# talmolab/sleap

Hardware: NVIDIA H100
Metric: frames/sec (1024x1024 bottom-up UNet+PAF) (higher is better)
Workload: dtype f16

## Files before the change

sleap_b200/csrc/sb_conv_tc.cu:

```cuda
#include <cuda.h>

#include <algorithm>

#include "sb_model.h"

namespace {

constexpr int TW = 16, TH = 8;
constexpr int MAX_GROUPS = 7, MAX_TAPS = 7;
constexpr size_t kMaxDynSmem = 225 * 1024;

struct TcTap { int row_off, w_tap; };
struct TcGroup { int dx, n_taps; TcTap taps[MAX_TAPS]; };

struct TcParams {
  int H, W;
  int tiles_x;
  int n_chunks, KC;
  int n_groups;
  TcGroup groups[MAX_GROUPS];
  int dy0, box_rows;
  int N, Cout;
  void* out;
  int out_f32, out_H, out_W, out_Ctot, out_coff;
// ... 466 lines not shown

  const int wg = warp >> 2;
  float acc[N / 2];
  const uint64_t desc_hi = make_desc(0, P.row_bytes, P.layout_type);
  const uint32_t a_row0 = (uint32_t)(wg * 64 * P.row_bytes);
  const uint32_t b_base = smem_u32(bank);
  mbar_wait(smem_u32(fullB), 0);
  int sa = 0;
  uint32_t pha = 0;
  for (int w = blockIdx.x; w < n_work; w += gridDim.x) {
    const int tile = w % P.n_tiles, b = w / P.n_tiles;
    const int x0 = (tile % P.tiles_x) * TW, y0 = (tile / P.tiles_x) * TH;
#pragma unroll
    for (int i = 0; i < N / 2; ++i) acc[i] = 0.f;
    int rel_a = -1, s = 0;
    uint32_t scale_d = 0;
    for (int ch = 0; ch < P.n_chunks; ++ch) {
      for (int g = 0; g < P.n_groups; ++g) {
        mbar_wait(smem_u32(fullA + sa), pha);
        const uint32_t a_base = smem_u32(a_ring + (size_t)sa * P.a_slot_bytes) + a_row0;
        const int n_taps = P.groups[g].n_taps;
        for (int t = 0; t < n_taps; ++t, ++s) {
          const uint64_t da = desc_hi + (uint64_t)((a_base + (uint32_t)(P.groups[g].taps[t].row_off * TW * P.row_bytes)) >> 4);
          const uint64_t db = desc_hi + (uint64_t)((b_base + (uint32_t)(s * P.b_slot_bytes)) >> 4);
          wgmma_fence();
          wgmma_reg_fence(acc);
#pragma unroll
          for (int k = 0; k < KSTEPS; ++k) {
            wgmma_f16<N>(acc, da + 2 * k, db + 2 * k, scale_d);
            scale_d = 1;
          }
          wgmma_commit();
          wgmma_reg_fence(acc);
          wgmma_wait<1>();
          __syncwarp();
          if (lane == 0 && rel_a >= 0) mbar_arrive(smem_u32(emptyA + rel_a));
          rel_a = t == n_taps - 1 ? sa : -1;
        }
        if (++sa == P.n_a_slots) { sa = 0; pha ^= 1; }
      }
    }
    wgmma_wait<0>();
    wgmma_reg_fence(acc);
    __syncwarp();
    if (lane == 0) mbar_arrive(smem_u32(emptyA + rel_a));
    if (w != (int)blockIdx.x) consumer_sync();
    conv_epilogue<N>(P, s_par, s_stage, acc, x0, y0, 0, b, warp, lane);
  }
}

constexpr int kHaloCols = 18;
constexpr int halo_by(int n, int kc) { return n <= 32 && n * kc <= 1024 ? 2 : 1; }
constexpr int halo_plane(int n, int kc) { return (8 * halo_by(n, kc) + 2) * kHaloCols * 16; }
constexpr int kHaloThreads = 384;

template <int NP>
__device__ __forceinline__ void stage_halo_patch(const TcParams& P, uint32_t dst, int plane, int rows, int c0, int b, int ys, int xs,
                                                 int lid, int n_loaders) {
  const __half* in = reinterpret_cast<const __half*>(P.in);
  const int pl = lid % NP, c = c0 + pl * 8;
  const bool c_ok = c < P.in_C;
  const __half* in_c = in + (size_t)b * P.H * P.W * P.in_Ctot + c;
  const uint32_t d = dst + (uint32_t)(pl * plane);
  for (int p = lid / NP; p < rows * kHaloCols; p += n_loaders / NP) {
    const int y = ys + p / kHaloCols, x = xs + p % kHaloCols;
    const bool ok = c_ok && y >= 0 && y < P.H && x >= 0 && x < P.W;
    const __half* src = ok ? in_c + ((size_t)y * P.W + x) * P.in_Ctot : in;
    asm volatile("cp.async.cg.shared.global [%0], [%1], 16, %2;" ::"r"(d + (uint32_t)(p * 16)), "l"(src), "r"(ok ? 16 : 0) : "memory");
  }
}

__device__ __forceinline__ void quad_transpose(uint32_t& v0, uint32_t& v1, uint32_t& v2, uint32_t& v3, int t) {
  const bool o1 = t & 1, o2 = t & 2;
  uint32_t r = __shfl_xor_sync(0xffffffffu, o1 ? v0 : v1, 1);
  if (o1) v0 = r; else v1 = r;
  r = __shfl_xor_sync(0xffffffffu, o1 ? v2 : v3, 1);
  if (o1) v2 = r; else v3 = r;
  r = __shfl_xor_sync(0xffffffffu, o2 ? v0 : v2, 2);
  if (o2) v0 = r; else v2 = r;
  r = __shfl_xor_sync(0xffffffffu, o2 ? v1 : v3, 2);
  if (o2) v1 = r; else v3 = r;
}

__device__ __forceinline__ uint32_t hmax2_u32(uint32_t a, uint32_t b) {
  const __half2 m = __hmax2(*reinterpret_cast<const __half2*>(&a), *reinterpret_cast<const __half2*>(&b));
  return *reinterpret_cast<const uint32_t*>(&m);
}

__device__ __forceinline__ float2 lds_f2(uint32_t saddr) {
  float2 v;
  asm("ld.shared.v2.f32 {%0, %1}, [%2];" : "=f"(v.x), "=f"(v.y) : "r"(saddr));
  return v;
}

template <int N>
__device__ __forceinline__ void frag_rows_f16(const float (&acc)[N / 2], uint32_t s_bias, int t, float lo, uint32_t (&hv)[N / 4]) {
  constexpr int NJ = N / 8;
#pragma unroll
  for (int j = 0; j < NJ; ++j) {
    const float2 bb = lds_f2(s_bias + 4u * (8 * j + 2 * t));
#pragma unroll
    for (int r = 0; r < 2; ++r) {
      const __half2 h2 = __floats2half2_rn(fmaxf(acc[4 * j + 2 * r] + bb.x, lo), fmaxf(acc[4 * j + 2 * r + 1] + bb.y, lo));
      hv[r * NJ + j] = *reinterpret_cast<const uint32_t*>(&h2);
    }
  }
}

template <int N>
__device__ __forceinline__ void frag_rows_store(uint32_t (&hv)[N / 4], __half* po, size_t row_step, bool ok0, bool ok1, int t) {
  constexpr int NJ = N / 8;
#pragma unroll
  for (int c0 = 0; c0 < 2 * NJ; c0 += 4) {
    quad_transpose(hv[c0], hv[c0 + 1], hv[c0 + 2], hv[c0 + 3], t);
    const int c = c0 + t, r = c / NJ, j = c % NJ;
    if (r ? ok1 : ok0) *reinterpret_cast<uint4*>(po + r * row_step + 8 * j) = make_uint4(hv[c0], hv[c0 + 1], hv[c0 + 2], hv[c0 + 3]);
  }
}

template <int N>
__device__ __forceinline__ void halo_block_epilogue(const TcParams& P, const float (&acc)[N / 2], uint32_t s_bias, int n0, int b,
                                                    int y, int x, int g, int t, float lo) {
  constexpr int NJ = N / 8;
  uint32_t hv[2 * NJ];
  frag_rows_f16<N>(acc, s_bias, t, lo, hv);
  if (P.pool_out != nullptr) {
    constexpr int NJ4 = (NJ + 3) / 4 * 4;
    uint32_t pv[NJ4];
#pragma unroll
    for (int j = 0; j < NJ4; ++j) {
      if (j < NJ) {
        const uint32_t m0 = hmax2_u32(hv[j], __shfl_xor_sync(0xffffffffu, hv[j], 4));
        const uint32_t m1 = hmax2_u32(hv[NJ + j], __shfl_xor_sync(0xffffffffu, hv[NJ + j], 4));
        pv[j] = hmax2_u32(m0, m1);
      } else {
        pv[j] = 0u;
      }
    }
    __half* pp = reinterpret_cast<__half*>(P.pool_out) + (((size_t)b * P.pool_H + (y >> 1)) * P.pool_W + (x >> 1)) * P.pool_Ctot +
                 P.pool_coff + n0;
    const bool st = (g & 1) == 0 && y < P.H && x < P.W;
#pragma unroll
    for (int c0 = 0; c0 < NJ4; c0 += 4) {
      quad_transpose(pv[c0], pv[c0 + 1], pv[c0 + 2], pv[c0 + 3], t);
      if (st && c0 + t < NJ) *reinterpret_cast<uint4*>(pp + 8 * (c0 + t)) = make_uint4(pv[c0], pv[c0 + 1], pv[c0 + 2], pv[c0 + 3]);
    }
  }
  if (!P.skip_out) {
    __half* po = reinterpret_cast<__half*>(P.out) + (((size_t)b * P.out_H + y) * P.out_W + x) * P.out_Ctot + P.out_coff + n0;
    frag_rows_store<N>(hv, po, (size_t)P.out_W * P.out_Ctot, y < P.H && x < P.W, y + 1 < P.H && x < P.W, t);
  }
}

template <int KSTEPS, int N>
__global__ void __launch_bounds__(kHaloThreads, 1) k_conv_wg_h(const __grid_constant__ CUtensorMap mapA,
                                                               const __grid_constant__ CUtensorMap mapB,
                                                               const __grid_constant__ TcParams P) {
  constexpr int BY = halo_by(N, 16 * KSTEPS), NB = 2 * BY;
  constexpr int NP = 2 * KSTEPS;
  constexpr int PH = 8 * BY + 2, PW = kHaloCols, PLANE = halo_plane(N, 16 * KSTEPS), SLOT = NP * PLANE;
  constexpr int kLoaders = kHaloThreads - kConsumerThreads;
  extern __shared__ __align__(1024) uint8_t smem_raw[];
  uint8_t* base = reinterpret_cast<uint8_t*>((reinterpret_cast<uintptr_t>(smem_raw) + 1023) & ~(uintptr_t)1023);
  uint8_t* bank = base;
  uint8_t* ring = bank + 9 * (size_t)P.b_slot_bytes;
  uint64_t* full = reinterpret_cast<uint64_t*>(ring + (size_t)P.n_a_slots * SLOT);
  uint64_t* empty = full + P.n_a_slots;
  uint64_t* fullB = empty + P.n_a_slots;
  float* s_bias = reinterpret_cast<float*>(fullB + 1);

  const int warp = threadIdx.x >> 5, lane = threadIdx.x & 31;
  const int tiles_x = (P.W + 15) / 16, n_tiles = tiles_x * ((P.H + 8 * BY - 1) / (8 * BY));
  const int n_work = n_tiles * P.batch;
  for (int i = threadIdx.x; i < N; i += blockDim.x) s_bias[i] = (P.bias && i < P.Cout) ? P.bias[i] : 0.f;
  if (threadIdx.x == 0) {
    for (int i = 0; i < P.n_a_slots; ++i) { mbar_init(smem_u32(full + i), kLoaders); mbar_init(smem_u32(empty + i), 4); }
    mbar_init(smem_u32(fullB), 1);
    asm volatile("fence.mbarrier_init.release.cluster;" ::: "memory");
    asm volatile("prefetch.tensormap [%0];" ::"l"(&mapB) : "memory");
  }
  __syncthreads();

  if (warp < kLoaders / 32) {
    if (threadIdx.x == 0) {
      mbar_expect_tx(smem_u32(fullB), (uint32_t)(9 * P.b_tx_bytes));
      for (int kx = 0; kx < 3; ++kx)
        for (int ky = 0; ky < 3; ++ky)
          tma_load_3d(smem_u32(bank + (size_t)(kx * 3 + ky) * P.b_slot_bytes), &mapB, smem_u32(fullB), 0, 0, ky * 3 + kx);
    }
    griddep_wait();
    for (int i = 0, w = blockIdx.x; w < n_work; ++i, w += gridDim.x) {
      if (w + (int)gridDim.x >= n_work) griddep_launch();
      const int s = i % P.n_a_slots;
      mbar_wait(smem_u32(empty + s), ((i / P.n_a_slots) & 1) ^ 1);
      const int tile = w % n_tiles, b = w / n_tiles;
      stage_halo_patch<NP>(P, smem_u32(ring + (size_t)s * SLOT), PLANE, PH, 0, b, (tile / tiles_x) * (8 * BY) - 1,
                           (tile % tiles_x) * 16 - 1, threadIdx.x, kLoaders);
      asm volatile("cp.async.mbarrier.arrive.noinc.shared::cta.b64 [%0];" ::"r"(smem_u32(full + s)) : "memory");
    }
    asm volatile("cp.async.wait_all;" ::: "memory");
    return;
  }

  const int wg = (warp >> 2) - 1, q = warp & 3, g = lane >> 2, t = lane & 3;
  const float lo = P.relu ? 0.f : -INFINITY;
  const uint64_t desc_a = make_desc_interleave(0, PLANE, PW * 16);
  const uint64_t desc_b = make_desc(0, P.row_bytes, P.layout_type);
  const uint32_t b_base = smem_u32(bank);
  mbar_wait(smem_u32(fullB), 0);
  float acc[NB][N / 2];
  for (int i = wg, w = blockIdx.x + wg * (int)gridDim.x; w < n_work; i += 2, w += 2 * (int)gridDim.x) {
    const int s = i % P.n_a_slots;
    mbar_wait(smem_u32(full + s), (i / P.n_a_slots) & 1);
    asm volatile("fence.proxy.async.shared::cta;" ::: "memory");
    const uint32_t a_base = smem_u32(ring + (size_t)s * SLOT);
    wgmma_fence();
#pragma unroll
    for (int bk = 0; bk < NB; ++bk) wgmma_reg_fence(acc[bk]);
#pragma unroll
    for (int kx = 0; kx < 3; ++kx)
#pragma unroll
      for (int ky = 0; ky < 3; ++ky)
#pragma unroll
        for (int k = 0; k < KSTEPS; ++k) {
          const uint64_t db = desc_b + (uint64_t)((b_base + (uint32_t)((kx * 3 + ky) * P.b_slot_bytes)) >> 4) + 2 * k;
#pragma unroll
          for (int bk = 0; bk < NB; ++bk) {
            const uint32_t a = a_base + (uint32_t)(((8 * (bk >> 1) + ky) * PW + 8 * (bk & 1) + kx) * 16 + 2 * k * PLANE);
            wgmma_f16<N>(acc[bk], desc_a + (uint64_t)(a >> 4), db, (kx | ky | k) ? 1u : 0u);
          }
        }
    wgmma_commit();
#pragma unroll
    for (int bk = 0; bk < NB; ++bk) wgmma_reg_fence(acc[bk]);
    wgmma_wait<0>();
#pragma unroll
    for (int bk = 0; bk < NB; ++bk) wgmma_reg_fence(acc[bk]);
    __syncwarp();
    if (lane == 0) mbar_arrive(smem_u32(empty + s));

    const int tile = w % n_tiles, b = w / n_tiles;
    const int x0 = (tile % tiles_x) * 16, y0 = (tile / tiles_x) * (8 * BY);
#pragma unroll
    for (int bk = 0; bk < NB; ++bk)
      halo_block_epilogue<N>(P, acc[bk], smem_u32(s_bias), 0, b, y0 + 8 * (bk >> 1) + 2 * q, x0 + 8 * (bk & 1) + g, g, t, lo);
  }
}

constexpr int kWideThreads = 384;
constexpr int kWidePatchLoaders = 96;
constexpr int wide_by(int n) { return n <= 64 ? 4 : 2; }
constexpr int wide_plane(int n) { return (8 * wide_by(n) + 2) * kHaloCols * 16; }

template <int N>
__global__ void __launch_bounds__(kWideThreads, 1) k_conv_wg_hw(const __grid_constant__ CUtensorMap mapA,
                                                                const __grid_constant__ CUtensorMap mapB,
                                                                const __grid_constant__ TcParams P) {
  constexpr int BY = wide_by(N), NP = 8, PH = 8 * BY + 2, PW = kHaloCols, PLANE = wide_plane(N), SLOT = NP * PLANE;
  constexpr int WSLOT = N * 128;
  extern __shared__ __align__(1024) uint8_t smem_raw[];
  uint8_t* base = reinterpret_cast<uint8_t*>((reinterpret_cast<uintptr_t>(smem_raw) + 1023) & ~(uintptr_t)1023);
  uint8_t* wring = base;
  uint8_t* pring = wring + (size_t)P.n_b_slots * WSLOT;
  uint64_t* pfull = reinterpret_cast<uint64_t*>(pring + (size_t)P.n_a_slots * SLOT);
  uint64_t* pempty = pfull + P.n_a_slots;
  uint64_t* wfull = pempty + P.n_a_slots;
  uint64_t* wempty = wfull + P.n_b_slots;
  float* s_bias = reinterpret_cast<float*>(wempty + P.n_b_slots);

  const int warp = threadIdx.x >> 5, lane = threadIdx.x & 31;
  const int tiles_x = (P.W + 15) / 16, n_pt = tiles_x * ((P.H + 8 * BY - 1) / (8 * BY));
  const int n_nt = P.Cout / N, n_work = n_nt * n_pt * P.batch;
  for (int i = threadIdx.x; i < P.Cout; i += blockDim.x) s_bias[i] = P.bias ? P.bias[i] : 0.f;
  if (threadIdx.x == 0) {
    for (int i = 0; i < P.n_a_slots; ++i) { mbar_init(smem_u32(pfull + i), kWidePatchLoaders); mbar_init(smem_u32(pempty + i), 8); }
    for (int i = 0; i < P.n_b_slots; ++i) { mbar_init(smem_u32(wfull + i), 1); mbar_init(smem_u32(wempty + i), 8); }
    asm volatile("fence.mbarrier_init.release.cluster;" ::: "memory");
    asm volatile("prefetch.tensormap [%0];" ::"l"(&mapB) : "memory");
  }
  __syncthreads();

  if (warp < 4) {
    setmaxnreg_dec<56>();
    if (warp != 1) {
      griddep_wait();
      const int pid = (warp == 0 ? 0 : 32 * (warp - 1)) + lane;
      for (int i = 0, w = blockIdx.x; w < n_work; w += gridDim.x) {
        if (w + (int)gridDim.x >= n_work) griddep_launch();
        const int pt = (w / n_nt) % n_pt, b = w / (n_nt * n_pt);
        const int xs = (pt % tiles_x) * 16 - 1, ys = (pt / tiles_x) * (8 * BY) - 1;
        for (int ch = 0; ch < P.n_chunks; ++ch, ++i) {
          const int s = i % P.n_a_slots;
          mbar_wait(smem_u32(pempty + s), ((i / P.n_a_slots) & 1) ^ 1);
          stage_halo_patch<NP>(P, smem_u32(pring + (size_t)s * SLOT), PLANE, PH, ch * 64, b, ys, xs, pid, kWidePatchLoaders);
          asm volatile("cp.async.mbarrier.arrive.noinc.shared::cta.b64 [%0];" ::"r"(smem_u32(pfull + s)) : "memory");
        }
      }
      asm volatile("cp.async.wait_all;" ::: "memory");
    } else if (warp == 1 && lane == 0) {
      for (int j = 0, w = blockIdx.x; w < n_work; w += gridDim.x) {
        const int n0 = (w % n_nt) * N;
        for (int ch = 0; ch < P.n_chunks; ++ch)
          for (int kx = 0; kx < 3; ++kx)
            for (int ky = 0; ky < 3; ++ky, ++j) {
              const int s = j % P.n_b_slots;
              mbar_wait(smem_u32(wempty + s), ((j / P.n_b_slots) & 1) ^ 1);
              mbar_expect_tx(smem_u32(wfull + s), (uint32_t)WSLOT);
              tma_load_3d(smem_u32(wring + (size_t)s * WSLOT), &mapB, smem_u32(wfull + s), ch * 64, n0, ky * 3 + kx);
            }
      }
    }
    return;
  }

  setmaxnreg_inc<224>();
  const int cw = (warp >> 2) - 1, q = warp & 3, g = lane >> 2, t = lane & 3;
  const float lo = P.relu ? 0.f : -INFINITY;
  const uint64_t desc_a = make_desc_interleave(0, PLANE, PW * 16);
  const uint64_t desc_b = make_desc(0, 128, 1);
  const uint32_t p_base = smem_u32(pring) + (uint32_t)(cw * (BY / 2) * 8 * PW * 16), w_base = smem_u32(wring);
  float acc[BY][N / 2];
  int ps = 0, ws = 0;
  uint32_t pph = 0, wph = 0;
  for (int w = blockIdx.x; w < n_work; w += gridDim.x) {
    int rel_w = -1, rel_p = -1;
    for (int ch = 0; ch < P.n_chunks; ++ch) {
      mbar_wait(smem_u32(pfull + ps), pph);
      asm volatile("fence.proxy.async.shared::cta;" ::: "memory");
      const uint32_t a_base = p_base + (uint32_t)(ps * SLOT);
#pragma unroll
      for (int kx = 0; kx < 3; ++kx)
#pragma unroll
        for (int ky = 0; ky < 3; ++ky) {
          mbar_wait(smem_u32(wfull + ws), wph);
          const uint64_t db = desc_b + (uint64_t)((w_base + (uint32_t)(ws * WSLOT)) >> 4);
          wgmma_fence();
#pragma unroll
          for (int i = 0; i < BY; ++i) wgmma_reg_fence(acc[i]);
#pragma unroll
          for (int k = 0; k < 4; ++k)
#pragma unroll
            for (int i = 0; i < BY; ++i) {
              const uint32_t a = a_base + (uint32_t)(((8 * (i >> 1) + ky) * PW + 8 * (i & 1) + kx) * 16 + 2 * k * PLANE);
              wgmma_f16<N>(acc[i], desc_a + (uint64_t)(a >> 4), db + 2 * k, (ch | kx | ky | k) ? 1u : 0u);
            }
          wgmma_commit();
#pragma unroll
          for (int i = 0; i < BY; ++i) wgmma_reg_fence(acc[i]);
          wgmma_wait<1>();
          __syncwarp();
          if (lane == 0) {
            if (rel_w >= 0) mbar_arrive(smem_u32(wempty + rel_w));
            if (rel_p >= 0) mbar_arrive(smem_u32(pempty + rel_p));
          }
          rel_w = ws;
          rel_p = (kx == 2 && ky == 2) ? ps : -1;
          if (++ws == P.n_b_slots) { ws = 0; wph ^= 1; }
        }
      if (++ps == P.n_a_slots) { ps = 0; pph ^= 1; }
    }
    wgmma_wait<0>();
#pragma unroll
    for (int i = 0; i < BY; ++i) wgmma_reg_fence(acc[i]);
    __syncwarp();
    if (lane == 0) { mbar_arrive(smem_u32(wempty + rel_w)); mbar_arrive(smem_u32(pempty + rel_p)); }

    const int n0 = (w % n_nt) * N, pt = (w / n_nt) % n_pt, b = w / (n_nt * n_pt);
    const int x0 = (pt % tiles_x) * 16, y0 = (pt / tiles_x) * (8 * BY) + cw * (BY / 2) * 8;
#pragma unroll
    for (int i = 0; i < BY; ++i)
      halo_block_epilogue<N>(P, acc[i], smem_u32(s_bias + n0), n0, b, y0 + 8 * (i >> 1) + 2 * q, x0 + 8 * (i & 1) + g, g, t, lo);
  }
}

constexpr int kTconvBoxRows = 17;
constexpr int kTconvBox = kTconvBoxRows * 16 * 128;
struct TcPhases {
  int n_groups[4], dy0[4], oy_add[4], ox_add[4];
  TcGroup groups[4][2];
};

// ... 400 lines not shown
    const size_t smem = 1024  + (size_t)nb * F.P.N * 128 + (size_t)n_a * a_slot + (size_t)(2 * n_a + 2 * nb) * 8 +
                        (size_t)F.P.Cout * sizeof(float);
    if (smem <= kMaxDynSmem) { F.ok = 1; F.P.n_a_slots = n_a; F.P.n_b_slots = nb; F.smem = smem; }
  }
}

static void fit_ctas(sb_handle_s* h, TcForm& F, int f) {
  if (!F.ok) return;
  int nb = 0;
  if (cudaOccupancyMaxActiveBlocksPerMultiprocessor(&nb, form_kernel(f, F.P.KC, F.P.N), F.threads, F.smem) != cudaSuccess || nb < 1) {
    cudaGetLastError();
    F.ok = 0;
    return;
  }
  F.max_ctas = nb * h->sm_count;
}

static bool halo_shape(const TcParams& P) {
  if (P.epi_mode != 1 || P.res != nullptr || P.n_groups != 3 || P.dy0 != -1 || P.box_rows != TH + 2 || P.oy_mul != 1 ||
      P.oy_add != 0 || P.ox_mul != 1 || P.ox_add != 0)
    return false;
  for (int g = 0; g < 3; ++g) {
    if (P.groups[g].dx != g - 1 || P.groups[g].n_taps != 3) return false;
    for (int ky = 0; ky < 3; ++ky)
      if (P.groups[g].taps[ky].row_off != ky || P.groups[g].taps[ky].w_tap != 3 * ky + g) return false;
  }
  return true;
}

static bool halo_eligible(const TcLaunch& L) {
  const TcParams& P = L.forms[0].P;
  return L.grid.y == 1 && P.n_chunks == 1 && P.N <= 64 && halo_shape(P);
}

static int wide_n(const TcParams& P) { return std::min(P.N, 128); }
static bool wide_eligible(const TcParams& P) { return P.KC == 64 && P.Cout % wide_n(P) == 0 && halo_shape(P); }

static void setup_forms(sb_handle_s* h, TcLaunch& L, int total_steps) {
  const TcParams& P = L.forms[0].P;
  L.form = 0;
  for (int f = 1; f < kForms; ++f) {
    L.forms[f] = L.forms[0];
    L.forms[f].ok = 0;
  }
  if (TcForm& F = L.forms[3]; form_kernel(3, P.KC, wide_n(P)) && wide_eligible(P)) {
    F.threads = kWideThreads;
    F.P.N = wide_n(P);
    fit_weight_ring(F, 2, (size_t)8 * wide_plane(F.P.N));
    const int by = wide_by(F.P.N);
    F.n_items = (P.Cout / F.P.N) * ((P.W + 15) / 16) * ((P.H + 8 * by - 1) / (8 * by));
    fit_ctas(h, F, 3);
  }
  if (TcForm& F = L.forms[2]; form_kernel(2, P.KC, P.N) && halo_eligible(L)) {
    F.threads = kHaloThreads;
    for (int na = 8; na >= 4 && !F.ok; --na)
      if (conv_smem_halo(P, na) <= kMaxDynSmem) { F.ok = 1; F.P.n_a_slots = na; F.P.n_b_slots = 9; F.smem = conv_smem_halo(P, na); }
    const int by = halo_by(P.N, P.KC);
    F.n_items = ((P.W + 15) / 16) * ((P.H + 8 * by - 1) / (8 * by));
    fit_ctas(h, F, 2);
  }
  TcForm& F = L.forms[1];
  if (!form_kernel(1, P.KC, P.N) || L.grid.y != 1) return;
  const int bank = P.n_chunks * total_steps;
  for (size_t budget : {(size_t)113 * 1024, kMaxDynSmem}) {
    for (int na = 4; na >= 2 && !F.ok; --na)
      if (conv_smem_resident(P, na, bank) <= budget) { F.ok = 1; F.P.n_a_slots = na; F.P.n_b_slots = bank; F.smem = conv_smem_resident(P, na, bank); }
    if (F.ok) break;
  }
  F.n_items = P.n_tiles;
  fit_ctas(h, F, 1);
}

static bool res_fusable(const SbModel* m, size_t oi) {
  const SbOp& op = m->ops[oi];
  if (op.kind() != SB_OPK_CONV || !op.residual() || oi + 1 >= m->ops.size() || getenv("SB_DISABLE_RES_FUSION")) return false;
  const SbOp& add = m->ops[oi + 1];
  if (add.kind() != SB_OPK_ADD || !(add.flags() & SB_OPF_FUSED_ADD) || add.out_buf() != op.sum_buf() || add.out_coff() != op.sum_coff()) return false;
  const SbBuffer& rb = m->buffers[op.res_buf()];
  const SbBuffer& sb = m->buffers[op.sum_buf()];
  const SbBuffer& ob = m->buffers[op.out_buf()];
  return !rb.f32 && !sb.f32 && !ob.f32 && rb.C % 8 == 0 && op.res_coff() % 8 == 0 && sb.C % 8 == 0 && op.sum_coff() % 8 == 0 &&
         rb.H == ob.H && rb.W == ob.W && sb.H == ob.H && sb.W == ob.W && op.pool_buf() < 0 && !(op.flags() & (SB_OPF_BN | SB_OPF_RELU));
}

static CUresult encode_weights(EncodeTiledFn enc, const SbConvTcPlan* plan, int Cin, int n_wtaps, int KC, int box_n, CUtensorMap* map) {
  cuuint64_t dims[3] = {(cuuint64_t)Cin, (cuuint64_t)plan->Cout_pad, (cuuint64_t)n_wtaps};
  cuuint64_t strides[2] = {(cuuint64_t)Cin * 2, (cuuint64_t)plan->Cout_pad * Cin * 2};
  cuuint32_t box[3] = {(cuuint32_t)KC, (cuuint32_t)box_n, 1};
  cuuint32_t es[3] = {1, 1, 1};
  return enc(map, CU_TENSOR_MAP_DATA_TYPE_FLOAT16, 3, (void*)plan->w16, dims, strides, box, es, CU_TENSOR_MAP_INTERLEAVE_NONE,
             swz_for(KC), CU_TENSOR_MAP_L2_PROMOTION_L2_256B, CU_TENSOR_MAP_FLOAT_OOB_FILL_NONE);
}

static int make_launch(sb_handle_s* h, SbModel* m, const SbOp& op, SbConvTcPlan* plan, int n_groups,
                       const TcGroup* groups, int dy0, int extra_rows, int n_wtaps, int oy_mul, int oy_add,
                       int ox_mul, int ox_add, const SbTcView* view = nullptr, bool fuse_res = false,
                       std::vector<TcLaunch>* dst = nullptr) {
  EncodeTiledFn enc = get_encode();
  if (!enc) return sb_fail(h, SB_ERR_CUDA, "cuTensorMapEncodeTiled entry point not available");
  const SbBuffer& ib = view ? view->in : m->buffers[op.in_buf()];
  const SbBuffer& ob0 = view ? view->out : m->buffers[op.out_buf()];
  const SbBuffer& ob = fuse_res ? m->buffers[op.sum_buf()] : ob0;
  const int Cin = view ? view->in.C : op.in_C(), Cout = view ? view->Cout : op.out_C();
  const int in_coff = view ? 0 : op.in_coff(), out_coff = view ? view->out_coff : (fuse_res ? op.sum_coff() : op.out_coff());
  const int KC = Cin > 32 ? 64 : (Cin > 16 ? 32 : 16);
  const int sub = (!view && op.kind() == SB_OPK_CONV) ? op.stride() : 1;
  const int gH = sub > 1 ? ob.H : ib.H, gW = sub > 1 ? ob.W : ib.W;
  TcLaunch L;
  memset(&L, 0, sizeof(L));
  TcForm& F0 = L.forms[0];
  TcParams& P = F0.P;
  P.H = gH; P.W = gW;
  P.tiles_x = (gW + TW - 1) / TW;
  const int tiles_y = (gH + TH - 1) / TH;
  P.n_chunks = (Cin + KC - 1) / KC; P.KC = KC;
  P.n_groups = n_groups;
  for (int g = 0; g < n_groups; ++g) P.groups[g] = groups[g];
  P.dy0 = dy0; P.box_rows = TH + extra_rows;
  const int N = wg_n(std::min(plan->Cout_pad, 256));
  P.N = N; P.Cout = Cout;
  P.out = ob.dev; P.out_f32 = ob.f32; P.out_H = ob.H; P.out_W = ob.W; P.out_Ctot = ob.C; P.out_coff = out_coff;
  P.oy_mul = oy_mul; P.oy_add = oy_add; P.ox_mul = ox_mul; P.ox_add = ox_add;
  if (view) {
    P.bias = view->bias; P.bn_scale = view->bn_scale; P.bn_shift = view->bn_shift; P.relu = view->relu;
  } else {
    P.bias = op.b_off() >= 0 ? m->weights_dev + op.b_off() : nullptr;
    P.bn_scale = (op.flags() & SB_OPF_BN) ? m->weights_dev + op.bn_scale_off() : nullptr;
    P.bn_shift = (op.flags() & SB_OPF_BN) ? m->weights_dev + op.bn_shift_off() : nullptr;
    P.relu = (op.flags() & SB_OPF_RELU) ? 1 : 0;
  }
  P.res = nullptr;
  if (fuse_res) {
    const SbBuffer& rb = m->buffers[op.res_buf()];
    P.res = (const __half*)rb.dev; P.res_Ctot = rb.C; P.res_coff = op.res_coff();
    P.relu = (m->ops[&op - m->ops.data() + 1].flags() & SB_OPF_RELU) ? 1 : 0;
  }
  P.pool_out = nullptr;
  if (!view && op.kind() == SB_OPK_CONV && op.pool_buf() >= 0 && !ob.f32 && Cout % 16 == 0 &&
      m->buffers[op.pool_buf()].C % 8 == 0 && op.pool_coff() % 8 == 0 && ib.H % 2 == 0 && ib.W % 2 == 0) {
    const SbBuffer& pb = m->buffers[op.pool_buf()];
    P.pool_out = pb.dev; P.pool_H = pb.H; P.pool_W = pb.W; P.pool_Ctot = pb.C; P.pool_coff = op.pool_coff();
  }
  P.split = (m->precision == 2 && !ob.f32) ? 1 : 0;
  P.epi_mode = 0;
  if (!P.split && !ob.f32 && P.bn_scale == nullptr && Cout % 16 == 0 && plan->Cout_pad == Cout &&
      ob.C % 16 == 0 && out_coff % 16 == 0 && (P.pool_out == nullptr || (P.pool_Ctot % 16 == 0 && P.pool_coff % 16 == 0)))
    P.epi_mode = 1;
  P.row_bytes = KC * 2;
  P.layout_type = KC == 64 ? 1 : (KC == 32 ? 2 : 3);
  P.a_tx_bytes = P.box_rows * TW * KC * 2;
  P.b_tx_bytes = N * KC * 2;
  P.a_slot_bytes = (P.a_tx_bytes + 1023) / 1024 * 1024;
  P.b_slot_bytes = (P.b_tx_bytes + 1023) / 1024 * 1024;
  int total_steps = 0;
  for (int g = 0; g < n_groups; ++g) total_steps += groups[g].n_taps;
  const size_t stage_bytes = (size_t)128 * (stage_cols(N) + 4) * sizeof(float);
  const size_t ring_budget = 200 * 1024 - stage_bytes;
  P.n_a_slots = std::min(3, P.n_chunks * n_groups);
  P.n_b_slots = std::min(4, P.n_chunks * total_steps);
  while ((size_t)P.n_a_slots * P.a_slot_bytes + (size_t)P.n_b_slots * P.b_slot_bytes > ring_budget && P.n_b_slots > 2) P.n_b_slots--;
  while ((size_t)P.n_a_slots * P.a_slot_bytes + (size_t)P.n_b_slots * P.b_slot_bytes > ring_budget && P.n_a_slots > 2) P.n_a_slots--;
  F0.ok = 1;
  F0.threads = kConvThreads;
  F0.smem = conv_smem(P, P.n_a_slots, P.n_b_slots);
  if (F0.smem > kMaxDynSmem) return sb_fail(h, SB_ERR_INVALID, "conv tile needs %zu bytes of shared memory", F0.smem);
  L.grid = dim3(P.tiles_x * tiles_y, (plan->Cout_pad + N - 1) / N, 1 );
  {
    cuuint64_t dims[4] = {(cuuint64_t)Cin, (cuuint64_t)gW, (cuuint64_t)gH, (cuuint64_t)m->B};
    cuuint64_t strides[3] = {(cuuint64_t)ib.C * 2 * sub, (cuuint64_t)ib.W * ib.C * 2 * sub, (cuuint64_t)ib.H * ib.W * ib.C * 2};
    cuuint32_t box[4] = {(cuuint32_t)KC, (cuuint32_t)TW, (cuuint32_t)P.box_rows, 1};
    cuuint32_t es[4] = {1, 1, 1, 1};
    void* gptr = (void*)((__half*)ib.dev + in_coff);
    P.in = gptr; P.in_Ctot = ib.C; P.in_C = Cin;
    CUresult r = enc(&F0.mapA, CU_TENSOR_MAP_DATA_TYPE_FLOAT16, 4, gptr, dims, strides, box, es, CU_TENSOR_MAP_INTERLEAVE_NONE,
                     swz_for(KC), CU_TENSOR_MAP_L2_PROMOTION_L2_128B, CU_TENSOR_MAP_FLOAT_OOB_FILL_NONE);
    if (r != CUDA_SUCCESS) return sb_fail(h, SB_ERR_CUDA, "cuTensorMapEncodeTiled(A) failed: %d", (int)r);
  }
  if (CUresult r = encode_weights(enc, plan, Cin, n_wtaps, KC, N, &F0.mapB); r != CUDA_SUCCESS)
    return sb_fail(h, SB_ERR_CUDA, "cuTensorMapEncodeTiled(B) failed: %d", (int)r);
  P.n_tiles = (int)L.grid.x;
  setup_forms(h, L, total_steps);
  if (L.forms[3].ok)
    if (CUresult r = encode_weights(enc, plan, Cin, n_wtaps, KC, L.forms[3].P.N, &L.forms[3].mapB); r != CUDA_SUCCESS)
      return sb_fail(h, SB_ERR_CUDA, "cuTensorMapEncodeTiled(B, wide form) failed: %d", (int)r);
  (dst ? *dst : plan->launches).push_back(L);
  return 0;
}

static int setup_tconv_form(sb_handle_s* h, SbModel* m, const SbOp& op, SbConvTcPlan* plan) {
  if (plan->launches.size() != 4) return 0;
  TcForm& T = plan->launches[0].forms[kTconvForm];
  const TcParams& P0 = plan->launches[0].forms[0].P;
  T.threads = kWideThreads;
  T.P.N = std::min(P0.N, 128);
  if (!form_kernel(kTconvForm, P0.KC, T.P.N) || P0.Cout % T.P.N) return 0;
  for (int p = 0; p < 4; ++p) {
    const TcParams& P = plan->launches[p].forms[0].P;
    if (P.epi_mode != 1 || P.n_groups > 2 || P.dy0 < -1 || P.dy0 > 0) return 0;
    T.Q.n_groups[p] = P.n_groups; T.Q.dy0[p] = P.dy0; T.Q.oy_add[p] = P.oy_add; T.Q.ox_add[p] = P.ox_add;
    for (int g = 0; g < P.n_groups; ++g) {
      for (int t = 0; t < P.groups[g].n_taps; ++t)
        if (P.groups[g].taps[t].row_off < 0 || P.groups[g].taps[t].row_off > 1) return 0;
      T.Q.groups[p][g] = P.groups[g];
    }
  }
  fit_weight_ring(T, 4, kTconvBox);
  T.n_items = 4 * (P0.Cout / T.P.N) * ((P0.W + 15) / 16) * ((P0.H + 15) / 16);
  fit_ctas(h, T, kTconvForm);
  if (!T.ok) return 0;
  EncodeTiledFn enc = get_encode();
  {
    cuuint64_t dims[4] = {(cuuint64_t)P0.in_C, (cuuint64_t)P0.W, (cuuint64_t)P0.H, (cuuint64_t)m->B};
    cuuint64_t strides[3] = {(cuuint64_t)P0.in_Ctot * 2, (cuuint64_t)P0.W * P0.in_Ctot * 2, (cuuint64_t)P0.H * P0.W * P0.in_Ctot * 2};
    cuuint32_t box[4] = {64, 16, (cuuint32_t)kTconvBoxRows, 1};
    cuuint32_t es[4] = {1, 1, 1, 1};
    CUresult r = enc(&T.mapA, CU_TENSOR_MAP_DATA_TYPE_FLOAT16, 4, const_cast<void*>(P0.in), dims, strides, box, es,
                     CU_TENSOR_MAP_INTERLEAVE_NONE, CU_TENSOR_MAP_SWIZZLE_128B, CU_TENSOR_MAP_L2_PROMOTION_L2_128B,
                     CU_TENSOR_MAP_FLOAT_OOB_FILL_NONE);
    if (r != CUDA_SUCCESS) return sb_fail(h, SB_ERR_CUDA, "cuTensorMapEncodeTiled(A, fused tconv) failed: %d", (int)r);
  }
  if (CUresult r = encode_weights(enc, plan, op.in_C(), op.k() * op.k(), 64, T.P.N, &T.mapB); r != CUDA_SUCCESS)
    return sb_fail(h, SB_ERR_CUDA, "cuTensorMapEncodeTiled(B, fused tconv) failed: %d", (int)r);
  return 0;
}

int sb_conv_tc_view_prepare(sb_handle_s* h, SbModel* m, int op_index, const SbTcView& v, const std::vector<float>& w) {
  if (v.in.W < TW || v.in.H < TH + v.R - 1) return 0;
  SbConvTcPlan* plan = new SbConvTcPlan();
  int cp = (v.Cout + 15) / 16 * 16;
  if (cp > 256) cp = (cp + 255) / 256 * 256;
  plan->Cout_pad = cp;
  std::vector<__half> w16((size_t)v.R * v.S * cp * 16, __float2half(0.f));
  for (int t = 0; t < v.R * v.S; ++t)
    for (int co = 0; co < v.Cout; ++co)
      for (int c = 0; c < 16; ++c) w16[((size_t)t * cp + co) * 16 + c] = __float2half_rn(w[((size_t)t * v.Cout + co) * 16 + c]);
  cudaError_t e = cudaMalloc((void**)&plan->w16, w16.size() * sizeof(__half));
  if (e == cudaSuccess) e = cudaMemcpy(plan->w16, w16.data(), w16.size() * sizeof(__half), cudaMemcpyHostToDevice);
// ... 323 lines not shown
```

sleap_b200/csrc/sb_tc_prims.cuh:

```cuda
#pragma once

__device__ __forceinline__ uint32_t smem_u32(const void* p) { return (uint32_t)__cvta_generic_to_shared(p); }

__device__ __forceinline__ void mbar_init(uint32_t bar, uint32_t count) {
  asm volatile("mbarrier.init.shared::cta.b64 [%0], %1;" ::"r"(bar), "r"(count));
}
__device__ __forceinline__ void mbar_expect_tx(uint32_t bar, uint32_t bytes) {
  asm volatile("mbarrier.arrive.expect_tx.shared::cta.b64 _, [%0], %1;" ::"r"(bar), "r"(bytes) : "memory");
}
__device__ __forceinline__ bool mbar_try_wait(uint32_t bar, uint32_t parity) {
  uint32_t ok;
  asm volatile(
      "{\n\t.reg .pred p;\n\t"
      "mbarrier.try_wait.parity.shared::cta.b64 p, [%1], %2;\n\t"
      "selp.u32 %0, 1, 0, p;\n\t}"
      : "=r"(ok) : "r"(bar), "r"(parity) : "memory");
  return ok != 0;
}
__device__ __forceinline__ void mbar_wait(uint32_t bar, uint32_t parity) {
  for (uint32_t it = 0; !mbar_try_wait(bar, parity); ++it)
    if (it > (1u << 24)) __trap();
}
__device__ __forceinline__ void mbar_arrive(uint32_t bar) {
  asm volatile("mbarrier.arrive.shared::cta.b64 _, [%0];" ::"r"(bar) : "memory");
}
__device__ __forceinline__ void tma_load_4d(uint32_t dst, const CUtensorMap* map, uint32_t bar, int c0, int c1,
                                            int c2, int c3) {
  asm volatile(
      "cp.async.bulk.tensor.4d.shared::cluster.global.mbarrier::complete_tx::bytes [%0], [%1, {%3, %4, %5, %6}], [%2];"
      ::"r"(dst), "l"(map), "r"(bar), "r"(c0), "r"(c1), "r"(c2), "r"(c3) : "memory");
}
__device__ __forceinline__ void tma_load_3d(uint32_t dst, const CUtensorMap* map, uint32_t bar, int c0, int c1, int c2) {
  asm volatile(
      "cp.async.bulk.tensor.3d.shared::cluster.global.mbarrier::complete_tx::bytes [%0], [%1, {%3, %4, %5}], [%2];"
      ::"r"(dst), "l"(map), "r"(bar), "r"(c0), "r"(c1), "r"(c2) : "memory");
}

__device__ __forceinline__ uint64_t make_desc(uint32_t saddr, int row_bytes, int layout_type) {
  uint64_t d = 0;
  d |= (uint64_t)((saddr >> 4) & 0x3FFF);
  d |= (uint64_t)1 << 16;
  d |= (uint64_t)(((8 * row_bytes) >> 4) & 0x3FFF) << 32;
  d |= (uint64_t)layout_type << 62;
  return d;
}
__device__ __forceinline__ uint64_t make_desc_interleave(uint32_t saddr, uint32_t lbo, uint32_t sbo) {
  uint64_t d = 0;
  d |= (uint64_t)((saddr >> 4) & 0x3FFF);
  d |= (uint64_t)((lbo >> 4) & 0x3FFF) << 16;
  d |= (uint64_t)((sbo >> 4) & 0x3FFF) << 32;
  return d;
}

__device__ __forceinline__ void wgmma_fence() { asm volatile("wgmma.fence.sync.aligned;" ::: "memory"); }
__device__ __forceinline__ void wgmma_commit() { asm volatile("wgmma.commit_group.sync.aligned;" ::: "memory"); }
template <int N>
__device__ __forceinline__ void wgmma_wait() { asm volatile("wgmma.wait_group.sync.aligned %0;" ::"n"(N) : "memory"); }
template <int R>
__device__ __forceinline__ void wgmma_reg_fence(float (&d)[R]) {
#pragma unroll
  for (int i = 0; i < R; ++i) asm volatile("" : "+f"(d[i])::"memory");
}

template <int N>
__device__ __forceinline__ void wgmma_f16(float (&d)[N / 2], uint64_t a_desc, uint64_t b_desc, uint32_t scale_d);
template <>
__device__ __forceinline__ void wgmma_f16<16>(float (&d)[8], uint64_t a_desc, uint64_t b_desc, uint32_t scale_d) {
  asm volatile(
      "{\n\t.reg .pred p;\n\t"
      "setp.ne.b32 p, %10, 0;\n\t"
      "wgmma.mma_async.sync.aligned.m64n16k16.f32.f16.f16 "
      "{%0, %1, %2, %3, %4, %5, %6, %7}, "
      "%8, %9, p, 1, 1, 0, 0;\n\t}"
      : "+f"(d[0]), "+f"(d[1]), "+f"(d[2]), "+f"(d[3]), "+f"(d[4]), "+f"(d[5]), "+f"(d[6]), "+f"(d[7])
      : "l"(a_desc), "l"(b_desc), "r"(scale_d) : "memory");
}
template <>
__device__ __forceinline__ void wgmma_f16<32>(float (&d)[16], uint64_t a_desc, uint64_t b_desc, uint32_t scale_d) {
  asm volatile(
      "{\n\t.reg .pred p;\n\t"
      "setp.ne.b32 p, %18, 0;\n\t"
      "wgmma.mma_async.sync.aligned.m64n32k16.f32.f16.f16 "
      "{%0, %1, %2, %3, %4, %5, %6, %7, %8, %9, %10, %11, %12, %13, %14, %15}, "
      "%16, %17, p, 1, 1, 0, 0;\n\t}"
      : "+f"(d[0]), "+f"(d[1]), "+f"(d[2]), "+f"(d[3]), "+f"(d[4]), "+f"(d[5]), "+f"(d[6]), "+f"(d[7]), "+f"(d[8]), "+f"(d[9]), "+f"(d[10]), "+f"(d[11]), "+f"(d[12]), "+f"(d[13]), "+f"(d[14]), "+f"(d[15])
      : "l"(a_desc), "l"(b_desc), "r"(scale_d) : "memory");
}
template <>
// ... 94 lines not shown
```

Baseline: 4254.

## Load halo input patches with 5D TMA instead of cp.async loader warps

Replaces the per-thread cp.async halo-patch staging in the halo and wide conv kernels with a single 5D tensor-map TMA load per slot. Each load is tracked by expect_tx on the full barrier. The halo kernel drops its extra loader warps, shrinking from 384 threads to kConvThreads with a single producer warp. Patch tensor maps are encoded on the host using OOB zero fill for the borders. This cuts producer instruction overhead and frees threads and registers, but relies on the TMA box layout matching the interleaved wgmma descriptor layout.

New measurement: 4678, median of 6. +10.0%, better.

```diff
diff --git a/sleap_b200/csrc/sb_conv_tc.cu b/sleap_b200/csrc/sb_conv_tc.cu
--- a/sleap_b200/csrc/sb_conv_tc.cu
+++ b/sleap_b200/csrc/sb_conv_tc.cu
@@ -542,23 +542,6 @@
 constexpr int kHaloCols = 18;
 constexpr int halo_by(int n, int kc) { return n <= 32 && n * kc <= 1024 ? 2 : 1; }
 constexpr int halo_plane(int n, int kc) { return (8 * halo_by(n, kc) + 2) * kHaloCols * 16; }
-constexpr int kHaloThreads = 384;
-
-template <int NP>
-__device__ __forceinline__ void stage_halo_patch(const TcParams& P, uint32_t dst, int plane, int rows, int c0, int b, int ys, int xs,
-                                                 int lid, int n_loaders) {
-  const __half* in = reinterpret_cast<const __half*>(P.in);
-  const int pl = lid % NP, c = c0 + pl * 8;
-  const bool c_ok = c < P.in_C;
-  const __half* in_c = in + (size_t)b * P.H * P.W * P.in_Ctot + c;
-  const uint32_t d = dst + (uint32_t)(pl * plane);
-  for (int p = lid / NP; p < rows * kHaloCols; p += n_loaders / NP) {
-    const int y = ys + p / kHaloCols, x = xs + p % kHaloCols;
-    const bool ok = c_ok && y >= 0 && y < P.H && x >= 0 && x < P.W;
-    const __half* src = ok ? in_c + ((size_t)y * P.W + x) * P.in_Ctot : in;
-    asm volatile("cp.async.cg.shared.global [%0], [%1], 16, %2;" ::"r"(d + (uint32_t)(p * 16)), "l"(src), "r"(ok ? 16 : 0) : "memory");
-  }
-}
 
 __device__ __forceinline__ void quad_transpose(uint32_t& v0, uint32_t& v1, uint32_t& v2, uint32_t& v3, int t) {
   const bool o1 = t & 1, o2 = t & 2;
@@ -643,13 +626,11 @@
 }
 
 template <int KSTEPS, int N>
-__global__ void __launch_bounds__(kHaloThreads, 1) k_conv_wg_h(const __grid_constant__ CUtensorMap mapA,
+__global__ void __launch_bounds__(kConvThreads, 1) k_conv_wg_h(const __grid_constant__ CUtensorMap mapA,
                                                                const __grid_constant__ CUtensorMap mapB,
                                                                const __grid_constant__ TcParams P) {
   constexpr int BY = halo_by(N, 16 * KSTEPS), NB = 2 * BY;
-  constexpr int NP = 2 * KSTEPS;
-  constexpr int PH = 8 * BY + 2, PW = kHaloCols, PLANE = halo_plane(N, 16 * KSTEPS), SLOT = NP * PLANE;
-  constexpr int kLoaders = kHaloThreads - kConsumerThreads;
+  constexpr int PW = kHaloCols, PLANE = halo_plane(N, 16 * KSTEPS), SLOT = 2 * KSTEPS * PLANE;
   extern __shared__ __align__(1024) uint8_t smem_raw[];
   uint8_t* base = reinterpret_cast<uint8_t*>((reinterpret_cast<uintptr_t>(smem_raw) + 1023) & ~(uintptr_t)1023);
   uint8_t* bank = base;
@@ -664,35 +645,35 @@
   const int n_work = n_tiles * P.batch;
   for (int i = threadIdx.x; i < N; i += blockDim.x) s_bias[i] = (P.bias && i < P.Cout) ? P.bias[i] : 0.f;
   if (threadIdx.x == 0) {
-    for (int i = 0; i < P.n_a_slots; ++i) { mbar_init(smem_u32(full + i), kLoaders); mbar_init(smem_u32(empty + i), 4); }
+    for (int i = 0; i < P.n_a_slots; ++i) { mbar_init(smem_u32(full + i), 1); mbar_init(smem_u32(empty + i), 4); }
     mbar_init(smem_u32(fullB), 1);
     asm volatile("fence.mbarrier_init.release.cluster;" ::: "memory");
+    asm volatile("prefetch.tensormap [%0];" ::"l"(&mapA) : "memory");
     asm volatile("prefetch.tensormap [%0];" ::"l"(&mapB) : "memory");
   }
   __syncthreads();
 
-  if (warp < kLoaders / 32) {
-    if (threadIdx.x == 0) {
+  if (warp == kConsumerThreads / 32) {
+    if (lane == 0) {
       mbar_expect_tx(smem_u32(fullB), (uint32_t)(9 * P.b_tx_bytes));
       for (int kx = 0; kx < 3; ++kx)
         for (int ky = 0; ky < 3; ++ky)
           tma_load_3d(smem_u32(bank + (size_t)(kx * 3 + ky) * P.b_slot_bytes), &mapB, smem_u32(fullB), 0, 0, ky * 3 + kx);
-    }
-    griddep_wait();
-    for (int i = 0, w = blockIdx.x; w < n_work; ++i, w += gridDim.x) {
-      if (w + (int)gridDim.x >= n_work) griddep_launch();
-      const int s = i % P.n_a_slots;
-      mbar_wait(smem_u32(empty + s), ((i / P.n_a_slots) & 1) ^ 1);
-      const int tile = w % n_tiles, b = w / n_tiles;
-      stage_halo_patch<NP>(P, smem_u32(ring + (size_t)s * SLOT), PLANE, PH, 0, b, (tile / tiles_x) * (8 * BY) - 1,
-                           (tile % tiles_x) * 16 - 1, threadIdx.x, kLoaders);
-      asm volatile("cp.async.mbarrier.arrive.noinc.shared::cta.b64 [%0];" ::"r"(smem_u32(full + s)) : "memory");
-    }
-    asm volatile("cp.async.wait_all;" ::: "memory");
+      griddep_wait();
+      for (int i = 0, w = blockIdx.x; w < n_work; ++i, w += gridDim.x) {
+        if (w + (int)gridDim.x >= n_work) griddep_launch();
+        const int s = i % P.n_a_slots;
+        mbar_wait(smem_u32(empty + s), ((i / P.n_a_slots) & 1) ^ 1);
+        const int tile = w % n_tiles, b = w / n_tiles;
+        mbar_expect_tx(smem_u32(full + s), (uint32_t)SLOT);
+        tma_load_5d(smem_u32(ring + (size_t)s * SLOT), &mapA, smem_u32(full + s), 0, (tile % tiles_x) * 16 - 1,
+                    (tile / tiles_x) * (8 * BY) - 1, 0, b);
+      }
+    }
     return;
   }
 
-  const int wg = (warp >> 2) - 1, q = warp & 3, g = lane >> 2, t = lane & 3;
+  const int wg = warp >> 2, q = warp & 3, g = lane >> 2, t = lane & 3;
   const float lo = P.relu ? 0.f : -INFINITY;
   const uint64_t desc_a = make_desc_interleave(0, PLANE, PW * 16);
   const uint64_t desc_b = make_desc(0, P.row_bytes, P.layout_type);
@@ -702,7 +683,6 @@
   for (int i = wg, w = blockIdx.x + wg * (int)gridDim.x; w < n_work; i += 2, w += 2 * (int)gridDim.x) {
     const int s = i % P.n_a_slots;
     mbar_wait(smem_u32(full + s), (i / P.n_a_slots) & 1);
-    asm volatile("fence.proxy.async.shared::cta;" ::: "memory");
     const uint32_t a_base = smem_u32(ring + (size_t)s * SLOT);
     wgmma_fence();
 #pragma unroll
@@ -738,7 +718,6 @@
 }
 
 constexpr int kWideThreads = 384;
-constexpr int kWidePatchLoaders = 96;
 constexpr int wide_by(int n) { return n <= 64 ? 4 : 2; }
 constexpr int wide_plane(int n) { return (8 * wide_by(n) + 2) * kHaloCols * 16; }
 
@@ -746,7 +725,7 @@
 __global__ void __launch_bounds__(kWideThreads, 1) k_conv_wg_hw(const __grid_constant__ CUtensorMap mapA,
                                                                 const __grid_constant__ CUtensorMap mapB,
                                                                 const __grid_constant__ TcParams P) {
-  constexpr int BY = wide_by(N), NP = 8, PH = 8 * BY + 2, PW = kHaloCols, PLANE = wide_plane(N), SLOT = NP * PLANE;
+  constexpr int BY = wide_by(N), PW = kHaloCols, PLANE = wide_plane(N), SLOT = 8 * PLANE;
   constexpr int WSLOT = N * 128;
   extern __shared__ __align__(1024) uint8_t smem_raw[];
   uint8_t* base = reinterpret_cast<uint8_t*>((reinterpret_cast<uintptr_t>(smem_raw) + 1023) & ~(uintptr_t)1023);
@@ -763,18 +742,18 @@
   const int n_nt = P.Cout / N, n_work = n_nt * n_pt * P.batch;
   for (int i = threadIdx.x; i < P.Cout; i += blockDim.x) s_bias[i] = P.bias ? P.bias[i] : 0.f;
   if (threadIdx.x == 0) {
-    for (int i = 0; i < P.n_a_slots; ++i) { mbar_init(smem_u32(pfull + i), kWidePatchLoaders); mbar_init(smem_u32(pempty + i), 8); }
+    for (int i = 0; i < P.n_a_slots; ++i) { mbar_init(smem_u32(pfull + i), 1); mbar_init(smem_u32(pempty + i), 8); }
     for (int i = 0; i < P.n_b_slots; ++i) { mbar_init(smem_u32(wfull + i), 1); mbar_init(smem_u32(wempty + i), 8); }
     asm volatile("fence.mbarrier_init.release.cluster;" ::: "memory");
+    asm volatile("prefetch.tensormap [%0];" ::"l"(&mapA) : "memory");
     asm volatile("prefetch.tensormap [%0];" ::"l"(&mapB) : "memory");
   }
   __syncthreads();
 
   if (warp < 4) {
     setmaxnreg_dec<56>();
-    if (warp != 1) {
+    if (warp == 0 && lane == 0) {
       griddep_wait();
-      const int pid = (warp == 0 ? 0 : 32 * (warp - 1)) + lane;
       for (int i = 0, w = blockIdx.x; w < n_work; w += gridDim.x) {
         if (w + (int)gridDim.x >= n_work) griddep_launch();
         const int pt = (w / n_nt) % n_pt, b = w / (n_nt * n_pt);
@@ -782,11 +761,10 @@
         for (int ch = 0; ch < P.n_chunks; ++ch, ++i) {
           const int s = i % P.n_a_slots;
           mbar_wait(smem_u32(pempty + s), ((i / P.n_a_slots) & 1) ^ 1);
-          stage_halo_patch<NP>(P, smem_u32(pring + (size_t)s * SLOT), PLANE, PH, ch * 64, b, ys, xs, pid, kWidePatchLoaders);
-          asm volatile("cp.async.mbarrier.arrive.noinc.shared::cta.b64 [%0];" ::"r"(smem_u32(pfull + s)) : "memory");
+          mbar_expect_tx(smem_u32(pfull + s), (uint32_t)SLOT);
+          tma_load_5d(smem_u32(pring + (size_t)s * SLOT), &mapA, smem_u32(pfull + s), 0, xs, ys, ch * 8, b);
         }
       }
-      asm volatile("cp.async.wait_all;" ::: "memory");
     } else if (warp == 1 && lane == 0) {
       for (int j = 0, w = blockIdx.x; w < n_work; w += gridDim.x) {
         const int n0 = (w % n_nt) * N;
@@ -816,7 +794,6 @@
     int rel_w = -1, rel_p = -1;
     for (int ch = 0; ch < P.n_chunks; ++ch) {
       mbar_wait(smem_u32(pfull + ps), pph);
-      asm volatile("fence.proxy.async.shared::cta;" ::: "memory");
       const uint32_t a_base = p_base + (uint32_t)(ps * SLOT);
 #pragma unroll
       for (int kx = 0; kx < 3; ++kx)
@@ -1323,7 +1300,7 @@
     fit_ctas(h, F, 3);
   }
   if (TcForm& F = L.forms[2]; form_kernel(2, P.KC, P.N) && halo_eligible(L)) {
-    F.threads = kHaloThreads;
+    F.threads = kConvThreads;
     for (int na = 8; na >= 4 && !F.ok; --na)
       if (conv_smem_halo(P, na) <= kMaxDynSmem) { F.ok = 1; F.P.n_a_slots = na; F.P.n_b_slots = 9; F.smem = conv_smem_halo(P, na); }
     const int by = halo_by(P.N, P.KC);
@@ -1361,6 +1338,15 @@
   cuuint32_t es[3] = {1, 1, 1};
   return enc(map, CU_TENSOR_MAP_DATA_TYPE_FLOAT16, 3, (void*)plan->w16, dims, strides, box, es, CU_TENSOR_MAP_INTERLEAVE_NONE,
              swz_for(KC), CU_TENSOR_MAP_L2_PROMOTION_L2_256B, CU_TENSOR_MAP_FLOAT_OOB_FILL_NONE);
+}
+
+static CUresult encode_patches(EncodeTiledFn enc, const TcParams& P, int frames, int rows, CUtensorMap* map) {
+  cuuint64_t dims[5] = {8, (cuuint64_t)P.W, (cuuint64_t)P.H, (cuuint64_t)(P.in_C / 8), (cuuint64_t)frames};
+  cuuint64_t strides[4] = {(cuuint64_t)P.in_Ctot * 2, (cuuint64_t)P.W * P.in_Ctot * 2, 16, (cuuint64_t)P.H * P.W * P.in_Ctot * 2};
+  cuuint32_t box[5] = {8, kHaloCols, (cuuint32_t)rows, (cuuint32_t)(P.KC / 8), 1};
+  cuuint32_t es[5] = {1, 1, 1, 1, 1};
+  return enc(map, CU_TENSOR_MAP_DATA_TYPE_FLOAT16, 5, const_cast<void*>(P.in), dims, strides, box, es, CU_TENSOR_MAP_INTERLEAVE_NONE,
+             CU_TENSOR_MAP_SWIZZLE_NONE, CU_TENSOR_MAP_L2_PROMOTION_L2_128B, CU_TENSOR_MAP_FLOAT_OOB_FILL_NONE);
 }
 
 static int make_launch(sb_handle_s* h, SbModel* m, const SbOp& op, SbConvTcPlan* plan, int n_groups,
@@ -1451,9 +1437,15 @@
     return sb_fail(h, SB_ERR_CUDA, "cuTensorMapEncodeTiled(B) failed: %d", (int)r);
   P.n_tiles = (int)L.grid.x;
   setup_forms(h, L, total_steps);
-  if (L.forms[3].ok)
+  if (L.forms[2].ok)
+    if (CUresult r = encode_patches(enc, P, m->B, 8 * halo_by(P.N, KC) + 2, &L.forms[2].mapA); r != CUDA_SUCCESS)
+      return sb_fail(h, SB_ERR_CUDA, "cuTensorMapEncodeTiled(patches, halo form) failed: %d", (int)r);
+  if (L.forms[3].ok) {
+    if (CUresult r = encode_patches(enc, P, m->B, 8 * wide_by(L.forms[3].P.N) + 2, &L.forms[3].mapA); r != CUDA_SUCCESS)
+      return sb_fail(h, SB_ERR_CUDA, "cuTensorMapEncodeTiled(patches, wide form) failed: %d", (int)r);
     if (CUresult r = encode_weights(enc, plan, Cin, n_wtaps, KC, L.forms[3].P.N, &L.forms[3].mapB); r != CUDA_SUCCESS)
       return sb_fail(h, SB_ERR_CUDA, "cuTensorMapEncodeTiled(B, wide form) failed: %d", (int)r);
+  }
   (dst ? *dst : plan->launches).push_back(L);
   return 0;
 }
diff --git a/sleap_b200/csrc/sb_tc_prims.cuh b/sleap_b200/csrc/sb_tc_prims.cuh
--- a/sleap_b200/csrc/sb_tc_prims.cuh
+++ b/sleap_b200/csrc/sb_tc_prims.cuh
@@ -34,6 +34,12 @@
   asm volatile(
       "cp.async.bulk.tensor.3d.shared::cluster.global.mbarrier::complete_tx::bytes [%0], [%1, {%3, %4, %5}], [%2];"
       ::"r"(dst), "l"(map), "r"(bar), "r"(c0), "r"(c1), "r"(c2) : "memory");
+}
+__device__ __forceinline__ void tma_load_5d(uint32_t dst, const CUtensorMap* map, uint32_t bar, int c0, int c1, int c2, int c3,
+                                            int c4) {
+  asm volatile(
+      "cp.async.bulk.tensor.5d.shared::cluster.global.mbarrier::complete_tx::bytes [%0], [%1, {%3, %4, %5, %6, %7}], [%2];"
+      ::"r"(dst), "l"(map), "r"(bar), "r"(c0), "r"(c1), "r"(c2), "r"(c3), "r"(c4) : "memory");
 }
 
 __device__ __forceinline__ uint64_t make_desc(uint32_t saddr, int row_bytes, int layout_type) {
```
